# ModelTC/Dipoorlet

Measured on AMD Instinct MI355X. Metric: calibration images/sec (whole node) + achieved HBM GB/s, ResNet-50 ONNX N=1024, -A hist, higher is better.
Workload: dtype f32; 1 GPU; ResNet-50 ONNX activation set (T=123, 26598376 fp32 elems/img), -A hist --bins 2048, N=1024 per GPU in 32 batches of 32: range pass + histogram pass + percentile clip; device=AMD Radeon Graphics (gfx950:sramecc+:xnack-), hist_checksum_ok=True, world_size_seen_by_backend=1

## Files before the change

### dipoorlet_amd/csrc/calib_kernels.hip

```cpp
#include "common.hpp"

#pragma clang fp contract(off)

namespace {

__device__ __forceinline__ void minmax_commit(const MinMaxOp& op, uint32_t slot, float* s_mn, float* s_mx, uint32_t* s_nan,
                                              uint32_t* __restrict__ min_enc, uint32_t* __restrict__ max_enc,
                                              uint32_t* __restrict__ nan_flag) {
    float mn = wave_min(op.mn), mx = wave_max(op.mx);
    uint32_t nn = __any(op.nan) ? 1u : 0u;
    const int w = threadIdx.x / kWave;
    if ((threadIdx.x & (kWave - 1)) == 0) {
        s_mn[w] = mn;
        s_mx[w] = mx;
        s_nan[w] = nn;
    }
    __syncthreads();
    if (threadIdx.x == 0) {
#pragma unroll
        for (int j = 1; j < kBlock / kWave; ++j) {
            mn = fminf(mn, s_mn[j]);
            mx = fmaxf(mx, s_mx[j]);
            nn |= s_nan[j];
        }
        if (mn <= mx) {
            atomicMin(min_enc + slot, enc_f32(mn));
            atomicMax(max_enc + slot, enc_f32(mx));
        }
        if (nn) atomicOr(nan_flag + slot, 1u);
    }
    __syncthreads();
}

__global__ __launch_bounds__(kBlock) void k_minmax(const dpl_work_item* __restrict__ items,
                                                    const uint32_t* __restrict__ bb,
                                                    const float* const* __restrict__ segs,
                                                    uint32_t* __restrict__ min_enc, uint32_t* __restrict__ max_enc,
                                                    uint32_t* __restrict__ nan_flag) {
    __shared__ float s_mn[kBlock / kWave], s_mx[kBlock / kWave];
    __shared__ uint32_t s_nan[kBlock / kWave];
    uint32_t k0, k1;
    block_items(bb, k0, k1);
    for (uint32_t k = k0; k < k1; ++k) {
        const dpl_work_item it = items[k];
        MinMaxOp op{INFINITY, -INFINITY, 0u};
        stream_span(segs[it.seg] + it.offset, it.count, op);
        minmax_commit(op, it.slot, s_mn, s_mx, s_nan, min_enc, max_enc, nan_flag);
    }
}

__global__ void k_minmax_init(uint32_t* mn, uint32_t* mx, uint32_t* nan, int64_t n) {
    int64_t i = (int64_t)blockIdx.x * blockDim.x + threadIdx.x;
    if (i < n) {
        mn[i] = 0xFFFFFFFFu;
        mx[i] = 0u;
        nan[i] = 0u;
    }
}

__device__ __forceinline__ void minmax_decode(uint32_t mn, uint32_t mx, uint32_t nan, float& omn, float& omx) {
    const bool bad = nan != 0u || mn == 0xFFFFFFFFu;
    omn = bad ? NAN : dec_f32(mn);
    omx = bad ? NAN : dec_f32(mx);
}

__global__ void k_minmax_finalize(const uint32_t* mn, const uint32_t* mx, const uint32_t* nan, int64_t n,
                                  float* omn, float* omx) {
    int64_t i = (int64_t)blockIdx.x * blockDim.x + threadIdx.x;
    if (i < n) minmax_decode(mn[i], mx[i], nan[i], omn[i], omx[i]);
}

__global__ void k_minmax_encode(const float* mn, const float* mx, int64_t n, uint32_t* emn, uint32_t* emx,
                                uint32_t* nan) {
    int64_t i = (int64_t)blockIdx.x * blockDim.x + threadIdx.x;
    if (i < n) {
        const bool bad = (mn[i] != mn[i]) || (mx[i] != mx[i]);
        emn[i] = bad ? 0xFFFFFFFFu : enc_f32(mn[i]);
        emx[i] = bad ? 0u : enc_f32(mx[i]);
        nan[i] = bad ? 1u : 0u;
    }
}

__device__ __forceinline__ float hist_edge(int i, float step, float first) {
    return __fadd_rn(__fmul_rn((float)i, step), first);
}

template <bool kFast>
struct HistOp {
    uint32_t* lds;
    float first, last, step, inv, denom;
    int last_bin;
    float fbins;
    uint32_t nonzero;
    __device__ __forceinline__ void operator()(float x) {
        const float a = fabsf(x);
        const bool nz = (a != 0.0f);
        nonzero += nz;
        if (kFast) {
            if (nz && (a <= last)) {
                const int i = (int)__fmul_rn(a, inv);
                const uint32_t dec = (a < __fmul_rn((float)i, step)) ? 0xFFFFFFFCu : 0u;
                atomicAdd(reinterpret_cast<uint32_t*>(reinterpret_cast<char*>(lds) + (((uint32_t)i << 2) + dec)), 1u);
            }
            return;
        }
        int i;
        if (kFast) {
            i = (int)__fmul_rn(a, inv);
            i = i > last_bin ? last_bin : i;
            i -= (a < __fmul_rn((float)i, step)) ? 1 : 0;
        } else {
            i = (int)__fmul_rn(__fdiv_rn(__fsub_rn(a, first), denom), fbins);
            i = i > last_bin ? last_bin : i;
            i = i < 0 ? 0 : i;
            i -= (a < hist_edge(i, step, first)) ? 1 : 0;
            i += (i != last_bin && a >= hist_edge(i + 1, step, first)) ? 1 : 0;
        }
        if (nz && (a <= last)) atomicAdd(lds + i, 1u);
    }
};

template <bool kFast>
__device__ __forceinline__ void hist_op_init(HistOp<kFast>& op, const dpl_hist_range& r, int bins, uint32_t* lds) {
    op.lds = lds;
    op.first = r.first;
    op.last = r.last;
    op.step = r.step;
    op.inv = r.inv;
    op.denom = __fsub_rn(r.last, r.first);
    op.last_bin = bins - 1;
    op.fbins = (float)bins;
    op.nonzero = 0u;
}

struct HistLds {
    static __host__ __device__ uint32_t* s_nz(uint32_t* counters, int bins) { return counters + bins + 1; }
    static __host__ __device__ uint32_t* end(uint32_t* counters, int bins) { return s_nz(counters, bins) + kBlock / kWave; }
    static __host__ __device__ size_t bytes(int bins) { return ((size_t)bins + 1 + kBlock / kWave) * sizeof(uint32_t); }
};

template <class Count>
__device__ __forceinline__ void hist_flush(uint32_t nonzero, const dpl_work_item& it, const dpl_hist_range& r, int bins,
                                           Count* __restrict__ hist, uint32_t* lds, uint32_t* s_nz) {
    const uint32_t nzw = wave_sum(nonzero);
    if ((threadIdx.x & (kWave - 1)) == 0) s_nz[threadIdx.x / kWave] = nzw;
    __syncthreads();
    if (threadIdx.x == 0) {
        uint32_t nzb = 0;
        for (int k = 0; k < kBlock / kWave; ++k) nzb += s_nz[k];
        const uint32_t z = it.count - nzb;
        if (z) atomicAdd(lds + r.zero_bin, z);
        const uint32_t top = lds[bins];
        if (top) atomicAdd(lds + bins - 1, top);
    }
    __syncthreads();
    Count* __restrict__ out = hist + (uint64_t)it.slot * (uint64_t)bins;
    for (int b = threadIdx.x; b < bins; b += kBlock) {
        const uint32_t c = lds[b];
        if (c) {
            if constexpr (sizeof(Count) == 8)
                atomicAdd(reinterpret_cast<unsigned long long*>(out + b), (unsigned long long)c);
            else
                atomicAdd(out + b, c);
        }
    }
}

template <bool kFast>
__device__ __forceinline__ void hist_body(const dpl_work_item& it, const float* const* __restrict__ segs,
                                          const dpl_hist_range& r, int bins, uint64_t* __restrict__ hist,
                                          uint32_t* lds, uint32_t* s_nz) {
    HistOp<kFast> op;
    hist_op_init(op, r, bins, lds);
    stream_span(segs[it.seg] + it.offset, it.count, op);
    hist_flush(op.nonzero, it, r, bins, hist, lds, s_nz);
}

__global__ __launch_bounds__(kBlock) void k_abs_hist(const dpl_work_item* __restrict__ items,
                                                      const uint32_t* __restrict__ bb,
                                                      const float* const* __restrict__ segs,
                                                      const dpl_hist_range* __restrict__ ranges, int bins,
                                                      uint64_t* __restrict__ hist) {
    extern __shared__ __attribute__((aligned(16))) uint32_t lds[];
    uint32_t* s_nz = HistLds::s_nz(lds, bins);
    uint32_t k0, k1;
    block_items(bb, k0, k1);
    for (uint32_t k = k0; k < k1; ++k) {
        const dpl_work_item it = items[k];
        const dpl_hist_range r = ranges[it.slot];
        if (r.status != 0u) continue;
        for (int b = threadIdx.x; b <= bins; b += kBlock) lds[b] = 0u;
        __syncthreads();
        if (r.exact_div)
            hist_body<false>(it, segs, r, bins, hist, lds, s_nz);
        else
            hist_body<true>(it, segs, r, bins, hist, lds, s_nz);
        __syncthreads();
    }
}

__device__ __forceinline__ float py_max(float a, float b) { return (b > a) ? b : a; }
__device__ __forceinline__ float py_min(float a, float b) { return (b < a) ? b : a; }

__device__ __forceinline__ dpl_hist_range hist_range_of(float gmin, float gmax, int bins) {
    dpl_hist_range r;
    const float dmax = py_max(gmax, -gmin);
    float first = 0.0f, last = dmax;
    r.dmax = dmax;
    r.status = 0u;
    if (!(fabsf(last) <= 3.402823466e+38f) || last < first) r.status = 1u;
    if (first == last) {
        first = -0.5f;
        last = 0.5f;
    }
    const float delta = __fsub_rn(last, first);
    const float fb = (float)bins;
    r.first = first;
    r.last = last;
    r.step = __fdiv_rn(delta, fb);
    r.inv = __fmul_rn(__fdiv_rn(fb, delta), 1.000001f);
    if (r.status == 0u) {
        const float e1 = hist_edge(1, r.step, first);
        const float el = hist_edge(bins - 1, r.step, first);
        const float el2 = hist_edge(bins - 2 > 0 ? bins - 2 : 0, r.step, first);
        if (!(r.step > 0.0f) || !(e1 > first) || !(last > el) || (bins > 2 && !(el > el2))) r.status = 2u;
    }
    r.exact_div = (first != 0.0f || !(fabsf(r.inv) <= 3.402823466e+38f) || r.step < 1.0e-30f) ? 1u : 0u;
    {
        const float a = 0.0f;
        float t = __fmul_rn(__fdiv_rn(__fsub_rn(a, first), delta), fb);
        int b = (int)t;
        b = b > bins - 1 ? bins - 1 : b;
        b = b < 0 ? 0 : b;
        if (a < hist_edge(b, r.step, first)) --b;
        if (b != bins - 1 && a >= hist_edge(b + 1, r.step, first)) ++b;
        r.zero_bin = (uint32_t)(b < 0 ? 0 : b);
    }
    return r;
}

__global__ void k_hist_prepare(const float* __restrict__ gmin, const float* __restrict__ gmax, int64_t n, int bins,
                               dpl_hist_range* __restrict__ out) {
    int64_t i = (int64_t)blockIdx.x * blockDim.x + threadIdx.x;
    if (i >= n) return;
    out[i] = hist_range_of(gmin[i], gmax[i], bins);
}

struct SpecEntry {
    dpl_hist_range* snap;
    uint32_t* flags;
    uint32_t* counts;
    SpecEntry(const void* d_entry, int64_t n_slots)
        : snap((dpl_hist_range*)d_entry), flags((uint32_t*)(snap + n_slots)), counts((uint32_t*)((char*)d_entry + counts_offset(n_slots))) {}
    static uint64_t counts_offset(int64_t n_slots) {
        return (((uint64_t)n_slots * (sizeof(dpl_hist_range) + sizeof(uint32_t))) + 15ull) & ~15ull;
    }
    static uint64_t bytes(int64_t n_slots, int bins) { return counts_offset(n_slots) + (uint64_t)n_slots * (uint64_t)bins * sizeof(uint32_t); }
};

__global__ __launch_bounds__(kBlock) void k_hist_snapshot(const uint32_t* __restrict__ mn, const uint32_t* __restrict__ mx,
                                                           const uint32_t* __restrict__ nan, int64_t n, int bins,
                                                           dpl_hist_range* __restrict__ snap, uint32_t* __restrict__ flags,
                                                           uint32_t* __restrict__ counts) {
    const int64_t i = (int64_t)blockIdx.x * blockDim.x + threadIdx.x;
    const int64_t stride = (int64_t)gridDim.x * blockDim.x;
    if (i < n) {
        float gmin, gmax;
        minmax_decode(mn[i], mx[i], nan[i], gmin, gmax);
        snap[i] = hist_range_of(gmin, gmax, bins);
        flags[i] = 0u;
    }
    const int64_t total = n * (int64_t)bins;
    for (int64_t j = i; j < total; j += stride) counts[j] = 0u;
}

template <bool kFast>
struct MinMaxHistOp {
    MinMaxOp m;
    HistOp<kFast> h;
    __device__ __forceinline__ void operator()(float x) {
        m(x);
        h(x);
    }
};

template <bool kFast>
__device__ __forceinline__ void minmax_hist_body(const dpl_work_item& it, const float* const* __restrict__ segs,
                                                 const dpl_hist_range& r, int bins, uint32_t* __restrict__ counts,
                                                 uint32_t* lds, uint32_t* s_nz, MinMaxOp& m) {
    MinMaxHistOp<kFast> op;
    op.m = m;
    hist_op_init(op.h, r, bins, lds);
    stream_span(segs[it.seg] + it.offset, it.count, op);
    m = op.m;
    hist_flush(op.h.nonzero, it, r, bins, counts, lds, s_nz);
}

struct MinMaxHistLds {
    static __host__ __device__ float* s_mn(uint32_t* base, int bins) { return reinterpret_cast<float*>(HistLds::end(base, bins)); }
    static __host__ __device__ float* s_mx(uint32_t* base, int bins) { return s_mn(base, bins) + kBlock / kWave; }
    static __host__ __device__ uint32_t* s_nan(uint32_t* base, int bins) {
        return reinterpret_cast<uint32_t*>(s_mx(base, bins) + kBlock / kWave);
    }
    static __host__ __device__ size_t bytes(int bins) { return HistLds::bytes(bins) + 3 * (kBlock / kWave) * sizeof(uint32_t); }
};

__global__ __launch_bounds__(kBlock) void k_minmax_hist(const dpl_work_item* __restrict__ items,
                                                         const uint32_t* __restrict__ bb,
                                                         const float* const* __restrict__ segs,
                                                         uint32_t* __restrict__ min_enc, uint32_t* __restrict__ max_enc,
                                                         uint32_t* __restrict__ nan_flag,
                                                         const dpl_hist_range* __restrict__ snap, int bins,
                                                         uint32_t* __restrict__ counts) {
    extern __shared__ __attribute__((aligned(16))) uint32_t lds_mh[];
    uint32_t* s_nz = HistLds::s_nz(lds_mh, bins);
    float* s_mn = MinMaxHistLds::s_mn(lds_mh, bins);
    float* s_mx = MinMaxHistLds::s_mx(lds_mh, bins);
    uint32_t* s_nan = MinMaxHistLds::s_nan(lds_mh, bins);
    uint32_t k0, k1;
    block_items(bb, k0, k1);
    for (uint32_t k = k0; k < k1; ++k) {
        const dpl_work_item it = items[k];
        const dpl_hist_range r = snap[it.slot];
        MinMaxOp m{INFINITY, -INFINITY, 0u};
        if (r.status != 0u) {
            stream_span(segs[it.seg] + it.offset, it.count, m);
        } else {
            for (int b = threadIdx.x; b <= bins; b += kBlock) lds_mh[b] = 0u;
            __syncthreads();
            if (r.exact_div)
                minmax_hist_body<false>(it, segs, r, bins, counts, lds_mh, s_nz, m);
            else
                minmax_hist_body<true>(it, segs, r, bins, counts, lds_mh, s_nz, m);
        }
        minmax_commit(m, it.slot, s_mn, s_mx, s_nan, min_enc, max_enc, nan_flag);
    }
}

__global__ __launch_bounds__(kBlock) void k_hist_resolve(const dpl_hist_range* __restrict__ snap,
                                                          const dpl_hist_range* __restrict__ fin,
                                                          const uint32_t* __restrict__ counts, const uint64_t* __restrict__ elems,
                                                          int bins, uint64_t* __restrict__ hist, uint32_t* __restrict__ flags,
                                                          unsigned long long* __restrict__ stats) {
    const uint32_t t = blockIdx.x;
    const uint32_t* a = reinterpret_cast<const uint32_t*>(snap + t);
    const uint32_t* b = reinterpret_cast<const uint32_t*>(fin + t);
    bool same = true;
#pragma unroll
    for (int w = 0; w < (int)(sizeof(dpl_hist_range) / 4); ++w) same = same && (a[w] == b[w]);
    const uint32_t status = fin[t].status;
    const bool valid = same && status == 0u;
    if (threadIdx.x == 0) {
        flags[t] = valid ? 1u : (status != 0u ? 2u : 0u);
        if (stats) {
            const unsigned long long e = elems[t];
            atomicAdd(stats + 0, 1ull);
            atomicAdd(stats + 2, e);
            if (valid) {
                atomicAdd(stats + 1, 1ull);
                atomicAdd(stats + 3, e);
            }
        }
    }
    if (!valid) return;
    const uint32_t* __restrict__ row = counts + (uint64_t)t * (uint64_t)bins;
    uint64_t* __restrict__ out = hist + (uint64_t)t * (uint64_t)bins;
    for (int j = threadIdx.x; j < bins; j += kBlock) {
        const uint32_t c = row[j];
        if (c) out[j] += (uint64_t)c;
    }
}

__device__ __forceinline__ uint64_t shfl_up_u64(uint64_t v, int d) {
    const uint32_t lo = __shfl_up((uint32_t)v, d, kWave), hi = __shfl_up((uint32_t)(v >> 32), d, kWave);
    return ((uint64_t)hi << 32) | lo;
}

__device__ __forceinline__ void rest_prefix(const uint64_t* __restrict__ elems, const uint32_t* __restrict__ flags, int n_tensors,
                                            uint64_t* P, uint64_t* s_tot) {
    const int per = (n_tensors + kBlock - 1) / kBlock;
    const int t0 = (int)threadIdx.x * per;
    uint64_t mine = 0;
    for (int j = 0; j < per; ++j) {
        const int t = t0 + j;
        if (t < n_tensors && flags[t] == 0u) mine += elems[t];
    }
    uint64_t incl = mine;
    const int lane = threadIdx.x & (kWave - 1), wv = threadIdx.x / kWave;
#pragma unroll
    for (int o = 1; o < kWave; o <<= 1) {
        const uint64_t up = shfl_up_u64(incl, o);
        if (lane >= o) incl += up;
    }
    if (lane == kWave - 1) s_tot[wv] = incl;
    __syncthreads();
    uint64_t run = incl - mine;
    for (int w = 0; w < wv; ++w) run += s_tot[w];
    for (int j = 0; j < per; ++j) {
        const int t = t0 + j;
        if (t < n_tensors) {
            P[t] = run;
            if (flags[t] == 0u) run += elems[t];
        }
    }
    if (threadIdx.x == kBlock - 1) P[n_tensors] = run;
    __syncthreads();
}

__device__ __forceinline__ void rest_cut(const uint64_t* P, int n_tensors, uint64_t G, uint64_t b, uint64_t& cut, int& at) {
    const uint64_t total = P[n_tensors], q = total / G, rem = total % G;
    const uint64_t target = (b >= G) ? total : q * b + (rem * b) / G;
    if (target >= total) {
        cut = total;
        at = n_tensors;
        return;
    }
    int lo = 1, hi = n_tensors;
    while (lo < hi) {
        const int mid = (lo + hi) >> 1;
        if (P[mid] > target) hi = mid; else lo = mid + 1;
    }
    at = lo - 1;
    cut = P[lo - 1] + ((target - P[lo - 1]) & ~1023ull);
}

struct RestPrefixLds {
    static __host__ __device__ uint64_t* P(uint32_t* base) { return reinterpret_cast<uint64_t*>(base); }
    static __host__ __device__ uint64_t* s_tot(uint32_t* base, int n_tensors) { return P(base) + n_tensors + 1; }
    static __host__ __device__ size_t bytes(int64_t n_tensors) { return ((size_t)n_tensors + 1 + kBlock / kWave) * sizeof(uint64_t); }
};

struct RestLds {
    static __host__ __device__ uint32_t* counters(uint32_t* base, int n_tensors) {
        return reinterpret_cast<uint32_t*>(RestPrefixLds::s_tot(base, n_tensors) + kBlock / kWave);
    }
    static __host__ __device__ size_t bytes(int64_t n_tensors, int bins) { return RestPrefixLds::bytes(n_tensors) + HistLds::bytes(bins); }
};

__global__ __launch_bounds__(kBlock) void k_abs_hist_rest(const uint64_t* __restrict__ elems, const uint32_t* __restrict__ flags,
                                                           int n_tensors, const float* const* __restrict__ segs,
                                                           const dpl_hist_range* __restrict__ ranges, int bins,
                                                           uint64_t* __restrict__ hist) {
    extern __shared__ __attribute__((aligned(16))) uint32_t lds_rest[];
    uint64_t* P = RestPrefixLds::P(lds_rest);
    uint64_t* s_tot = RestPrefixLds::s_tot(lds_rest, n_tensors);
    uint32_t* lds = RestLds::counters(lds_rest, n_tensors);
    uint32_t* s_nz = HistLds::s_nz(lds, bins);
    rest_prefix(elems, flags, n_tensors, P, s_tot);
    if (P[n_tensors] == 0) return;
    uint64_t cut[2];
    int at[2];
    rest_cut(P, n_tensors, gridDim.x, blockIdx.x, cut[0], at[0]);
    rest_cut(P, n_tensors, gridDim.x, (uint64_t)blockIdx.x + 1, cut[1], at[1]);
    uint64_t pos = cut[0];
    const uint64_t end = cut[1];
    int t = at[0];
    while (pos < end) {
        while (P[t + 1] <= pos) ++t;
        const uint64_t stop = P[t + 1] < end ? P[t + 1] : end;
        dpl_work_item it;
        it.offset = pos - P[t];
        it.count = (uint32_t)(stop - pos);
        it.seg = (uint32_t)t;
        it.slot = (uint32_t)t;
        it.reserved = 0u;
        const dpl_hist_range r = ranges[t];
        for (int b = threadIdx.x; b <= bins; b += kBlock) lds[b] = 0u;
        __syncthreads();
        if (r.exact_div)
            hist_body<false>(it, segs, r, bins, hist, lds, s_nz);
        else
            hist_body<true>(it, segs, r, bins, hist, lds, s_nz);
        __syncthreads();
        pos = stop;
    }
}

__global__ __launch_bounds__(kBlock) void k_hist_spec_cuts(const uint64_t* __restrict__ elems, const uint32_t* __restrict__ flags,
                                                            int n_tensors, uint64_t* __restrict__ cuts) {
    extern __shared__ __attribute__((aligned(16))) uint32_t lds_cuts[];
    uint64_t* P = RestPrefixLds::P(lds_cuts);
    uint64_t* s_tot = RestPrefixLds::s_tot(lds_cuts, n_tensors);
    rest_prefix(elems, flags, n_tensors, P, s_tot);
    if (threadIdx.x != 0) return;
    uint64_t cut = 0;
    int at = 0;
    if (P[n_tensors] != 0) rest_cut(P, n_tensors, gridDim.x, blockIdx.x, cut, at);
    cuts[blockIdx.x] = cut;
    if (blockIdx.x + 1 == gridDim.x) cuts[gridDim.x] = P[n_tensors];
}

__device__ __forceinline__ void store_bin_clip(int found, float gmin, float gmax, int bins, float* __restrict__ clip) {
    float lo = gmin, hi = gmax;
    if (found >= 0) {
        const float dmax = py_max(-gmin, gmax);
        const float cv = __fmul_rn((float)found + 0.5f, __fdiv_rn(dmax, (float)bins));
        lo = py_max(-cv, gmin);
        hi = py_min(cv, gmax);
    }
    clip[0] = lo;
    clip[1] = hi;
}

__global__ __launch_bounds__(kWave) void k_hist_percentile(const uint64_t* __restrict__ hist,
                                                            const float* __restrict__ gmin_a,
                                                            const float* __restrict__ gmax_a, int bins,
                                                            double threshold, float* __restrict__ clip) {
    const int slot = blockIdx.x;
    const int lane = threadIdx.x;
    const uint64_t* h = hist + (uint64_t)slot * bins;
    unsigned long long tot = 0;
    for (int b = lane; b < bins; b += kWave) tot += h[b];
#pragma unroll
    for (int o = 32; o > 0; o >>= 1) tot += __shfl_xor(tot, o, kWave);
    const double total = (double)(long long)tot;
    const float gmin = gmin_a[slot], gmax = gmax_a[slot];
    double accum = 0.0;
    int found = -1;
    uint64_t raw_next = lane < bins ? h[lane] : 0ull;
    for (int base = 0; base < bins && found < 0; base += kWave) {
        const int b = base + lane;
        const double hv = (b < bins) ? (double)(float)(long long)raw_next / total : 0.0;
        raw_next = (b + kWave < bins) ? h[b + kWave] : 0ull;
        const int lim = (bins - base) < kWave ? (bins - base) : kWave;
        const int h_lo = __double2loint(hv), h_hi = __double2hiint(hv);
        uint64_t reached = 0;
        if (lim == kWave) {
#pragma unroll
            for (int j = 0; j < kWave; ++j) {
                accum += __hiloint2double(__builtin_amdgcn_readlane(h_hi, j), __builtin_amdgcn_readlane(h_lo, j));
                reached |= (accum >= threshold) ? (1ull << j) : 0ull;
            }
        } else {
            for (int j = 0; j < lim; ++j) {
                accum += __hiloint2double(__builtin_amdgcn_readlane(h_hi, j), __builtin_amdgcn_readlane(h_lo, j));
                reached |= (accum >= threshold) ? (1ull << j) : 0ull;
            }
        }
        if (reached) found = base + __builtin_ctzll(reached);
    }
    if (lane == 0) store_bin_clip(found, gmin, gmax, bins, clip + 2 * slot);
}

constexpr double kKlEps = 1e-4;

__device__ __forceinline__ uint32_t kl_live_below(const uint64_t* __restrict__ mask, const uint32_t* __restrict__ bcnt, uint32_t x) {
    const uint32_t k = x >> 6;
    return bcnt[k] + (uint32_t)__popcll(mask[k] & ((1ull << (x & 63u)) - 1ull));
}

struct KlLds {
    static __host__ __device__ uint32_t nblk(int bins) { return ((uint32_t)bins + 63u) >> 6; }
    static __host__ __device__ uint64_t* mask(uint64_t* cs, int bins) { return cs + bins + 1; }
    static __host__ __device__ uint64_t* part(uint64_t* cs, int bins) { return mask(cs, bins) + nblk(bins) + 1; }
    static __host__ __device__ uint32_t* bcnt(uint64_t* cs, int bins) { return reinterpret_cast<uint32_t*>(part(cs, bins) + kBlock); }
    static __host__ __device__ size_t bytes(int bins) {
        return ((size_t)bins + 1 + nblk(bins) + 1 + kBlock) * sizeof(uint64_t) + ((size_t)nblk(bins) + 1) * sizeof(uint32_t);
    }
};

__global__ __launch_bounds__(kBlock) void k_hist_kl(const uint64_t* __restrict__ hist, int bins, int levels, int n_chunks,
                                                     double* __restrict__ div) {
    extern __shared__ __attribute__((aligned(16))) uint64_t kl_lds[];
    const uint32_t nblk = KlLds::nblk(bins);
    uint64_t* cs = kl_lds;
    uint64_t* mask = KlLds::mask(kl_lds, bins);
    uint64_t* part = KlLds::part(kl_lds, bins);
    uint32_t* bcnt = KlLds::bcnt(kl_lds, bins);
    const uint32_t tid = threadIdx.x, lane = tid & (kWave - 1), wave = tid / kWave;
    const uint32_t slot = blockIdx.x / (uint32_t)n_chunks, chunk = blockIdx.x % (uint32_t)n_chunks;
    const uint64_t* __restrict__ h = hist + (uint64_t)slot * (uint64_t)bins;
    double* __restrict__ out = div + (uint64_t)slot * ((uint64_t)bins + 1u);
    const uint32_t L = (uint32_t)levels, C = (uint32_t)n_chunks, nb = (uint32_t)bins;

    {
        const uint32_t per = (nb + kBlock - 1) / kBlock;
        const uint32_t b0 = tid * per < nb ? tid * per : nb, b1 = b0 + per < nb ? b0 + per : nb;
        uint64_t s = 0;
        for (uint32_t b = b0; b < b1; ++b) s += h[b];
        part[tid] = s;
        for (uint32_t k = wave; k < nblk; k += kBlock / kWave) {
            const uint32_t b = k * kWave + lane;
            const uint64_t m = __ballot(b < nb && h[b] != 0ull);
            if (lane == 0) mask[k] = m;
        }
        if (tid == 0) mask[nblk] = 0ull;
        __syncthreads();
        uint64_t off = 0;
        for (uint32_t j = 0; j < (uint32_t)kBlock; ++j) off += j < tid ? part[j] : 0ull;
        for (uint32_t b = b0; b < b1; ++b) {
            cs[b] = off;
            off += h[b];
        }
        if (tid == kBlock - 1) cs[nb] = off;
        for (uint32_t k = tid; k <= nblk; k += kBlock) {
            uint32_t a = 0;
            for (uint32_t j = 0; j < nblk; ++j) a += j < k ? (uint32_t)__popcll(mask[j]) : 0u;
            bcnt[k] = a;
        }
        __syncthreads();
    }
    for (uint32_t i = chunk + tid * C; i < L; i += kBlock * C) out[i] = INFINITY;

    const uint64_t N = cs[nb];
    const double dN = (double)(long long)N;
    const uint32_t first = L + (chunk + C - L % C) % C;
    for (uint32_t i = first + wave * C; i <= nb; i += (kBlock / kWave) * C) {
        const uint64_t csi = cs[i];
        const uint64_t outl = N - csi;
        const uint32_t s_last = (uint32_t)(((uint64_t)(L - 1u) * i) / L);
        const uint32_t woke = (csi == cs[i - 1] && outl != 0ull) ? 1u : 0u;
        const uint32_t n1p = kl_live_below(mask, bcnt, i) + woke;
        const uint32_t n1q = n1p - ((csi == cs[s_last] && outl != 0ull) ? 1u : 0u);
        double res = INFINITY;
        if (n1p != 0u && n1q != 0u) {
            const uint32_t zp = i - n1p, zq = i - n1q;
            const double e1p = kKlEps * (double)zp / (double)n1p;
            const double e1q = kKlEps * (double)zq / (double)n1q;
            if (e1p < 1.0 && e1q < 1.0) {
                const double Sp = dN - (double)n1p * e1p + (double)zp * kKlEps;
                const double Sq = (double)(long long)csi - (double)n1q * e1q + (double)zq * kKlEps;
                double acc = 0.0;
                for (uint32_t b = lane; b < i; b += kWave) {
                    uint64_t pb = cs[b + 1] - cs[b];
                    if (b == i - 1u) pb += outl;
                    if (pb != 0ull) {
                        const uint32_t g = ((b + 1u) * L - 1u) / i;
                        const uint32_t s0 = (g * i) / L, s1 = ((g + 1u) * i) / L;
                        const uint64_t G = cs[s1] - cs[s0];
                        double qs = kKlEps;
                        if (G != 0ull) {
                            const uint32_t live = kl_live_below(mask, bcnt, s1) - kl_live_below(mask, bcnt, s0) + (s1 == i ? woke : 0u);
                            qs = (double)(long long)G / (double)live - e1q;
                        }
                        const double P = ((double)(long long)pb - e1p) / Sp, Q = qs / Sq;
                        acc += P * log(P / Q);
                    }
                }
                acc = wave_sum(acc);
                const double Pz = kKlEps / Sp, Qz = kKlEps / Sq;
                res = acc + (double)zp * (Pz * log(Pz / Qz));
            }
        }
        if (lane == 0) out[i] = res;
    }
}

__global__ __launch_bounds__(kWave) void k_hist_kl_pick(const double* __restrict__ div, const float* __restrict__ gmin_a,
                                                         const float* __restrict__ gmax_a, int bins, int32_t* __restrict__ best,
                                                         float* __restrict__ clip) {
    const int slot = blockIdx.x;
    const int lane = threadIdx.x;
    const double* __restrict__ d = div + (uint64_t)slot * ((uint64_t)bins + 1u);
    double bv = INFINITY;
    int bi = -1;
    for (int i = lane; i <= bins; i += kWave) {
        const double v = d[i];
        if (v < bv) {
            bv = v;
            bi = i;
        }
    }
#pragma unroll
    for (int o = 32; o > 0; o >>= 1) {
        const double ov = __shfl_xor(bv, o, kWave);
        const int oi = __shfl_xor(bi, o, kWave);
        if (ov < bv || (ov == bv && oi >= 0 && (bi < 0 || oi < bi))) {
            bv = ov;
            bi = oi;
        }
    }
    if (lane == 0) {
        best[slot] = bi;
        store_bin_clip(bi >= 0 ? bi - 1 : -1, gmin_a[slot], gmax_a[slot], bins, clip + 2 * slot);
    }
}

constexpr int kGridUniform = DPL_GRID_UNIFORM, kGridE4M3 = DPL_GRID_E4M3;

struct QmseLds {
    static __host__ __device__ uint64_t* part(double* hd, int bins) { return reinterpret_cast<uint64_t*>(hd + bins); }
    static __host__ __device__ size_t bytes(int bins) { return (size_t)bins * sizeof(double) + (kBlock / kWave) * sizeof(uint64_t); }
};

template <int GRID>
__global__ __launch_bounds__(kBlock) void k_hist_qmse(const uint64_t* __restrict__ hist, int bins, int first, int top, int n_chunks,
                                                       double* __restrict__ err) {
    extern __shared__ __attribute__((aligned(16))) double qm_lds[];
    double* hd = qm_lds;
    uint64_t* part = QmseLds::part(qm_lds, bins);
    const uint32_t tid = threadIdx.x, lane = tid & (kWave - 1), wave = tid / kWave;
    const uint32_t slot = blockIdx.x / (uint32_t)n_chunks, chunk = blockIdx.x % (uint32_t)n_chunks;
    const uint64_t* __restrict__ h = hist + (uint64_t)slot * (uint64_t)bins;
    double* __restrict__ out = err + (uint64_t)slot * ((uint64_t)bins + 1u);
    const uint32_t F = (uint32_t)first, C = (uint32_t)n_chunks, nb = (uint32_t)bins;

    uint64_t s = 0;
    for (uint32_t b = tid; b < nb; b += kBlock) {
        const uint64_t v = h[b];
        s += v;
        hd[b] = (double)(long long)v;
    }
#pragma unroll
    for (int o = 32; o > 0; o >>= 1) s += __shfl_xor(s, o, kWave);
    if (lane == 0) part[wave] = s;
    __syncthreads();
    uint64_t N = 0;
#pragma unroll
    for (int w = 0; w < kBlock / kWave; ++w) N += part[w];

    for (uint32_t i = chunk + tid * C; i < F; i += kBlock * C) out[i] = INFINITY;

    constexpr double unit = GRID == kGridE4M3 ? 512.0 : 1.0;
    const double dtop = GRID == kGridE4M3 ? 448.0 : (double)top;
    const double atop = unit * dtop;
    const double norm = (double)(long long)N * (4.0 * atop * atop);
    for (uint32_t i = F + chunk + wave * C; i <= nb; i += (kBlock / kWave) * C) {
        const double t = (double)(2u * i - 1u);
        const double rt = 1.0 / (unit * t);
        double acc = 0.0;
        if (N != 0ull) {
            for (uint32_t b = lane; b < nb; b += kWave) {
                const double hb = hd[b];
                if (hb != 0.0) {
                    const double a = (double)(2u * b + 1u) * atop;
                    const double v = fmin(a * rt, dtop);
                    double q;
                    if (GRID == kGridE4M3) {
                        int e = (int)((__double_as_longlong(v) >> 52) & 0x7FF) - 1023;
                        e = e < -6 ? -6 : e;
                        const double istep = __longlong_as_double((long long)(1023 + 3 - e) << 52);
                        const double step512 = __longlong_as_double((long long)(1023 + 9 - 3 + e) << 52);
                        q = rint(v * istep) * step512;
                    } else {
                        q = rint(v);
                    }
                    const double dt = a - q * t;
                    acc += hb * (dt * dt);
                }
            }
            acc = wave_sum(acc);
        }
        if (lane == 0) out[i] = N != 0ull ? acc / norm : INFINITY;
    }
}

inline int check_bins(const char* who, int bins) {
    if (bins < 1 || bins > DPL_MAX_BINS) {
        snprintf(g_err, sizeof(g_err), "%s: bins must be in [1, %d]", who, DPL_MAX_BINS);
        return -2;
    }
    return 0;
}

inline int check_spec_geometry(const char* who, int64_t n_slots, int64_t n_blocks) {
    const bool slots_ok = n_slots > 0 && n_slots <= DPL_HIST_SPEC_MAX_TENSORS;
    if (slots_ok && n_blocks > 0 && n_blocks <= 0x7FFFFFFFll) return 0;
    snprintf(g_err, sizeof(g_err), "%s: %s", who, slots_ok ? "n_blocks out of range" : "n_slots must be in [1, DPL_HIST_SPEC_MAX_TENSORS]");
    return -2;
}

inline int candidate_chunks(const char* who, int64_t n_slots, int64_t n_cand, int64_t& chunks) {
    chunks = (1024 + n_slots - 1) / n_slots;
    if (chunks > n_cand / 8) chunks = n_cand / 8;
    if (chunks < 1) chunks = 1;
    if (n_slots * chunks > 0x7FFFFFFFll) {
        snprintf(g_err, sizeof(g_err), "%s: too many slots", who);
        return -2;
    }
    return 0;
}

}

extern "C" {

int dpl_minmax_init(uint32_t* d_min_enc, uint32_t* d_max_enc, uint32_t* d_nan, int64_t n_slots, dpl_stream_t s) {
    if (n_slots <= 0) return 0;
    hipLaunchKernelGGL(k_minmax_init, dim3(grid_for(n_slots, 256)), dim3(256), 0, (hipStream_t)s, d_min_enc,
                       d_max_enc, d_nan, n_slots);
    DPL_LAUNCH_CHECK("k_minmax_init");
    return 0;
}

int dpl_minmax_accumulate(const dpl_work_item* d_items, int64_t n_items, const uint32_t* d_block_begin,
                          int64_t n_blocks, const float* const* d_seg_ptrs, uint32_t* d_min_enc,
                          uint32_t* d_max_enc, uint32_t* d_nan, dpl_stream_t s) {
    if (n_items <= 0) return 0;
    if (int e = check_blocks("dpl_minmax_accumulate", n_items, d_block_begin, n_blocks)) return e;
    hipLaunchKernelGGL(k_minmax, dim3((unsigned)n_blocks), dim3(kBlock), 0, (hipStream_t)s, d_items, d_block_begin,
                       d_seg_ptrs, d_min_enc, d_max_enc, d_nan);
    DPL_LAUNCH_CHECK("k_minmax");
    return 0;
}

int dpl_minmax_finalize(const uint32_t* d_min_enc, const uint32_t* d_max_enc, const uint32_t* d_nan,
                        int64_t n_slots, float* d_min, float* d_max, dpl_stream_t s) {
    if (n_slots <= 0) return 0;
    hipLaunchKernelGGL(k_minmax_finalize, dim3(grid_for(n_slots, 256)), dim3(256), 0, (hipStream_t)s, d_min_enc,
                       d_max_enc, d_nan, n_slots, d_min, d_max);
    DPL_LAUNCH_CHECK("k_minmax_finalize");
    return 0;
}

int dpl_minmax_encode(const float* d_min, const float* d_max, int64_t n_slots, uint32_t* d_min_enc,
                      uint32_t* d_max_enc, uint32_t* d_nan, dpl_stream_t s) {
    if (n_slots <= 0) return 0;
    hipLaunchKernelGGL(k_minmax_encode, dim3(grid_for(n_slots, 256)), dim3(256), 0, (hipStream_t)s, d_min, d_max,
                       n_slots, d_min_enc, d_max_enc, d_nan);
    DPL_LAUNCH_CHECK("k_minmax_encode");
    return 0;
}

int dpl_hist_prepare(const float* d_min, const float* d_max, int64_t n_slots, int bins, dpl_hist_range* d_ranges,
                     dpl_stream_t s) {
    if (int e = check_bins("dpl_hist_prepare", bins)) return e;
    if (n_slots <= 0) return 0;
    hipLaunchKernelGGL(k_hist_prepare, dim3(grid_for(n_slots, 64)), dim3(64), 0, (hipStream_t)s, d_min, d_max,
                       n_slots, bins, d_ranges);
    DPL_LAUNCH_CHECK("k_hist_prepare");
    return 0;
}

int dpl_abs_hist_accumulate(const dpl_work_item* d_items, int64_t n_items, const uint32_t* d_block_begin,
                            int64_t n_blocks, const float* const* d_seg_ptrs, const dpl_hist_range* d_ranges,
                            int bins, uint64_t* d_hist, dpl_stream_t s) {
    if (int e = check_bins("dpl_abs_hist_accumulate", bins)) return e;
    if (n_items <= 0) return 0;
    if (int e = check_blocks("dpl_abs_hist_accumulate", n_items, d_block_begin, n_blocks)) return e;
    hipLaunchKernelGGL(k_abs_hist, dim3((unsigned)n_blocks), dim3(kBlock), HistLds::bytes(bins), (hipStream_t)s, d_items,
                       d_block_begin, d_seg_ptrs, d_ranges, bins, d_hist);
    DPL_LAUNCH_CHECK("k_abs_hist");
    return 0;
}

uint64_t dpl_hist_spec_entry_bytes(int64_t n_slots, int bins) {
    if (n_slots < 0 || bins < 1 || bins > DPL_MAX_BINS) return 0;
    return SpecEntry::bytes(n_slots, bins);
}

int dpl_minmax_hist_accumulate(const dpl_work_item* d_items, int64_t n_items, const uint32_t* d_block_begin,
                               int64_t n_blocks, const float* const* d_seg_ptrs, uint32_t* d_min_enc, uint32_t* d_max_enc,
                               uint32_t* d_nan, int64_t n_slots, int bins, void* d_entry, dpl_stream_t s) {
    if (int e = check_bins("dpl_minmax_hist_accumulate", bins)) return e;
    if (!d_entry || ((uintptr_t)d_entry & 15u)) return fail_msg("dpl_minmax_hist_accumulate: d_entry must be 16-byte aligned");
    if (n_slots <= 0 || n_slots > 0x7FFFFFFFll) return fail_msg("dpl_minmax_hist_accumulate: n_slots out of range");
    if (n_items <= 0) return 0;
    if (int e = check_blocks("dpl_minmax_hist_accumulate", n_items, d_block_begin, n_blocks)) return e;
    const SpecEntry entry(d_entry, n_slots);
    int64_t zb = grid_for(n_slots * (int64_t)bins, kBlock * 8);
    if (zb < grid_for(n_slots, kBlock)) zb = grid_for(n_slots, kBlock);
    if (zb > 1024) zb = 1024;
    hipLaunchKernelGGL(k_hist_snapshot, dim3((unsigned)zb), dim3(kBlock), 0, (hipStream_t)s, d_min_enc, d_max_enc, d_nan,
                       n_slots, bins, entry.snap, entry.flags, entry.counts);
    DPL_LAUNCH_CHECK("k_hist_snapshot");
    hipLaunchKernelGGL(k_minmax_hist, dim3((unsigned)n_blocks), dim3(kBlock), MinMaxHistLds::bytes(bins), (hipStream_t)s, d_items,
                       d_block_begin, d_seg_ptrs, d_min_enc, d_max_enc, d_nan, entry.snap, bins, entry.counts);
    DPL_LAUNCH_CHECK("k_minmax_hist");
    return 0;
}

int dpl_hist_spec_accumulate(void* d_entry, const uint64_t* d_elems, int64_t n_slots, int64_t n_blocks,
                             const float* const* d_seg_ptrs, const dpl_hist_range* d_ranges, int bins, uint64_t* d_hist,
                             uint64_t* d_stats, dpl_stream_t s) {
    if (int e = check_bins("dpl_hist_spec_accumulate", bins)) return e;
    if (!d_entry || ((uintptr_t)d_entry & 15u)) return fail_msg("dpl_hist_spec_accumulate: d_entry must be 16-byte aligned");
    if (int e = check_spec_geometry("dpl_hist_spec_accumulate", n_slots, n_blocks)) return e;
    const SpecEntry entry(d_entry, n_slots);
    hipLaunchKernelGGL(k_hist_resolve, dim3((unsigned)n_slots), dim3(kBlock), 0, (hipStream_t)s, entry.snap, d_ranges, entry.counts,
                       d_elems, bins, d_hist, entry.flags, (unsigned long long*)d_stats);
    DPL_LAUNCH_CHECK("k_hist_resolve");
    hipLaunchKernelGGL(k_abs_hist_rest, dim3((unsigned)n_blocks), dim3(kBlock), RestLds::bytes(n_slots, bins), (hipStream_t)s, d_elems,
                       entry.flags, (int)n_slots, d_seg_ptrs, d_ranges, bins, d_hist);
    DPL_LAUNCH_CHECK("k_abs_hist_rest");
    return 0;
}

int dpl_hist_spec_cuts(const void* d_entry, const uint64_t* d_elems, int64_t n_slots, int64_t n_blocks, uint64_t* d_cuts,
                       dpl_stream_t s) {
    if (!d_entry || !d_cuts) return fail_msg("dpl_hist_spec_cuts: null argument");
    if (int e = check_spec_geometry("dpl_hist_spec_cuts", n_slots, n_blocks)) return e;
    hipLaunchKernelGGL(k_hist_spec_cuts, dim3((unsigned)n_blocks), dim3(kBlock), RestPrefixLds::bytes(n_slots), (hipStream_t)s, d_elems,
                       SpecEntry(d_entry, n_slots).flags, (int)n_slots, d_cuts);
    DPL_LAUNCH_CHECK("k_hist_spec_cuts");
    return 0;
}

int dpl_hist_percentile(const uint64_t* d_hist, const float* d_min, const float* d_max, int64_t n_slots, int bins,
                        double threshold, float* d_clip, dpl_stream_t s) {
    if (n_slots <= 0) return 0;
    hipLaunchKernelGGL(k_hist_percentile, dim3((unsigned)n_slots), dim3(kWave), 0, (hipStream_t)s, d_hist, d_min,
                       d_max, bins, threshold, d_clip);
    DPL_LAUNCH_CHECK("k_hist_percentile");
    return 0;
}

int dpl_hist_kl(const uint64_t* d_hist, const float* d_min, const float* d_max, int64_t n_slots, int bins, int levels,
                double* d_div, int32_t* d_best, float* d_clip, dpl_stream_t s) {
    if (int e = check_bins("dpl_hist_kl", bins)) return e;
    if (levels < 2 || levels > bins) return fail_msg("dpl_hist_kl: levels must be in [2, bins]");
    if (n_slots <= 0) return 0;
    int64_t chunks;
    if (int e = candidate_chunks("dpl_hist_kl", n_slots, (int64_t)bins - levels + 1, chunks)) return e;
    hipLaunchKernelGGL(k_hist_kl, dim3((unsigned)(n_slots * chunks)), dim3(kBlock), KlLds::bytes(bins), (hipStream_t)s, d_hist, bins,
                       levels, (int)chunks, d_div);
    DPL_LAUNCH_CHECK("k_hist_kl");
    hipLaunchKernelGGL(k_hist_kl_pick, dim3((unsigned)n_slots), dim3(kWave), 0, (hipStream_t)s, d_div, d_min, d_max, bins,
                       d_best, d_clip);
    DPL_LAUNCH_CHECK("k_hist_kl_pick");
    return 0;
}

int dpl_hist_qmse(const uint64_t* d_hist, const float* d_min, const float* d_max, int64_t n_slots, int bins, int first, int grid,
                  int top, double* d_err, int32_t* d_best, float* d_clip, dpl_stream_t s) {
    if (int e = check_bins("dpl_hist_qmse", bins)) return e;
    if (first < 1 || first > bins) return fail_msg("dpl_hist_qmse: first must be in [1, bins]");
    if (grid != DPL_GRID_UNIFORM && grid != DPL_GRID_E4M3) return fail_msg("dpl_hist_qmse: grid must be DPL_GRID_UNIFORM or DPL_GRID_E4M3");
    if (grid == DPL_GRID_UNIFORM && (top < 1 || top > 32767)) return fail_msg("dpl_hist_qmse: top must be in [1, 32767] on the uniform grid");
    if (grid == DPL_GRID_E4M3 && top != 0) return fail_msg("dpl_hist_qmse: top must be 0 on the E4M3 grid (its largest value is 448)");
    if (n_slots <= 0) return 0;
    int64_t chunks;
    if (int e = candidate_chunks("dpl_hist_qmse", n_slots, (int64_t)bins - first + 1, chunks)) return e;
    const size_t lds = QmseLds::bytes(bins);
    const dim3 wgs((unsigned)(n_slots * chunks));
    if (grid == DPL_GRID_E4M3)
        hipLaunchKernelGGL(k_hist_qmse<kGridE4M3>, wgs, dim3(kBlock), lds, (hipStream_t)s, d_hist, bins, first, top, (int)chunks, d_err);
    else
        hipLaunchKernelGGL(k_hist_qmse<kGridUniform>, wgs, dim3(kBlock), lds, (hipStream_t)s, d_hist, bins, first, top, (int)chunks, d_err);
    DPL_LAUNCH_CHECK("k_hist_qmse");
    hipLaunchKernelGGL(k_hist_kl_pick, dim3((unsigned)n_slots), dim3(kWave), 0, (hipStream_t)s, d_err, d_min, d_max, bins,
                       d_best, d_clip);
    DPL_LAUNCH_CHECK("k_hist_kl_pick");
    return 0;
}

}
```

Baseline: 58750 images/s.

## Fuse speculative histogram resolve into rest-histogram kernel, batch row adds

Merges the per-tensor resolve kernel into the rest-histogram kernel. Each block now recomputes the snapshot-versus-final verdict inline for the prefix sum, adds validated speculative count rows in a grid-stride loop, and then processes its share of unresolved data. This drops one kernel launch and the dependency between the two kernels. Row accumulation is batched with 8 loads in flight per thread. The cost is that every block re-reads all snapshot and range records during the prefix, and the rest histogram work now waits behind each block's share of row adds.

Measured after the change: 59030 images/s (median of 2 runs). Within noise of the previous version (+0.5%).

```diff
diff --git a/dipoorlet_amd/csrc/calib_kernels.hip b/dipoorlet_amd/csrc/calib_kernels.hip
--- a/dipoorlet_amd/csrc/calib_kernels.hip
+++ b/dipoorlet_amd/csrc/calib_kernels.hip
@@ -337,37 +337,35 @@
     }
 }
 
-__global__ __launch_bounds__(kBlock) void k_hist_resolve(const dpl_hist_range* __restrict__ snap,
-                                                          const dpl_hist_range* __restrict__ fin,
-                                                          const uint32_t* __restrict__ counts, const uint64_t* __restrict__ elems,
-                                                          int bins, uint64_t* __restrict__ hist, uint32_t* __restrict__ flags,
-                                                          unsigned long long* __restrict__ stats) {
-    const uint32_t t = blockIdx.x;
+__device__ __forceinline__ uint32_t spec_verdict(const dpl_hist_range* __restrict__ snap, const dpl_hist_range* __restrict__ fin,
+                                                 uint32_t t) {
     const uint32_t* a = reinterpret_cast<const uint32_t*>(snap + t);
     const uint32_t* b = reinterpret_cast<const uint32_t*>(fin + t);
-    bool same = true;
-#pragma unroll
-    for (int w = 0; w < (int)(sizeof(dpl_hist_range) / 4); ++w) same = same && (a[w] == b[w]);
+    uint32_t diff = 0u;
+#pragma unroll
+    for (int w = 0; w < (int)(sizeof(dpl_hist_range) / 4); ++w) diff |= a[w] ^ b[w];
     const uint32_t status = fin[t].status;
-    const bool valid = same && status == 0u;
-    if (threadIdx.x == 0) {
-        flags[t] = valid ? 1u : (status != 0u ? 2u : 0u);
-        if (stats) {
-            const unsigned long long e = elems[t];
-            atomicAdd(stats + 0, 1ull);
-            atomicAdd(stats + 2, e);
-            if (valid) {
-                atomicAdd(stats + 1, 1ull);
-                atomicAdd(stats + 3, e);
-            }
-        }
-    }
-    if (!valid) return;
-    const uint32_t* __restrict__ row = counts + (uint64_t)t * (uint64_t)bins;
-    uint64_t* __restrict__ out = hist + (uint64_t)t * (uint64_t)bins;
-    for (int j = threadIdx.x; j < bins; j += kBlock) {
-        const uint32_t c = row[j];
-        if (c) out[j] += (uint64_t)c;
+    return status != 0u ? 2u : (diff == 0u ? 1u : 0u);
+}
+
+constexpr int kRowTrip = 8;
+__device__ __forceinline__ void spec_add_row(const uint32_t* __restrict__ row, uint64_t* __restrict__ out, int bins) {
+    for (int base = (int)threadIdx.x; base < bins; base += kBlock * kRowTrip) {
+        uint32_t c[kRowTrip];
+        uint64_t h[kRowTrip];
+#pragma unroll
+        for (int k = 0; k < kRowTrip; ++k) {
+            const int j = base + k * kBlock, jj = j < bins ? j : bins - 1;
+            c[k] = row[jj];
+            h[k] = out[jj];
+        }
+#pragma unroll
+        for (int k = 0; k < kRowTrip; ++k) asm volatile("" : "+v"(c[k]), "+v"(h[k]));
+#pragma unroll
+        for (int k = 0; k < kRowTrip; ++k) {
+            const int j = base + k * kBlock;
+            if (j < bins && c[k]) out[j] = h[k] + (uint64_t)c[k];
+        }
     }
 }
 
@@ -376,14 +374,20 @@
     return ((uint64_t)hi << 32) | lo;
 }
 
-__device__ __forceinline__ void rest_prefix(const uint64_t* __restrict__ elems, const uint32_t* __restrict__ flags, int n_tensors,
-                                            uint64_t* P, uint64_t* s_tot) {
+template <class ToRead>
+__device__ __forceinline__ void rest_prefix(const uint64_t* __restrict__ elems, int n_tensors, uint64_t* P, uint64_t* s_tot,
+                                            ToRead to_read) {
     const int per = (n_tensors + kBlock - 1) / kBlock;
     const int t0 = (int)threadIdx.x * per;
     uint64_t mine = 0;
     for (int j = 0; j < per; ++j) {
         const int t = t0 + j;
-        if (t < n_tensors && flags[t] == 0u) mine += elems[t];
+        if (t < n_tensors) {
+            const uint64_t e = elems[t];
+            const uint64_t share = to_read(t) ? e : 0ull;
+            P[t] = share;
+            mine += share;
+        }
     }
     uint64_t incl = mine;
     const int lane = threadIdx.x & (kWave - 1), wv = threadIdx.x / kWave;
@@ -399,8 +403,9 @@
     for (int j = 0; j < per; ++j) {
         const int t = t0 + j;
         if (t < n_tensors) {
+            const uint64_t share = P[t];
             P[t] = run;
-            if (flags[t] == 0u) run += elems[t];
+            run += share;
         }
     }
     if (threadIdx.x == kBlock - 1) P[n_tensors] = run;
@@ -437,16 +442,33 @@
     static __host__ __device__ size_t bytes(int64_t n_tensors, int bins) { return RestPrefixLds::bytes(n_tensors) + HistLds::bytes(bins); }
 };
 
-__global__ __launch_bounds__(kBlock) void k_abs_hist_rest(const uint64_t* __restrict__ elems, const uint32_t* __restrict__ flags,
-                                                           int n_tensors, const float* const* __restrict__ segs,
-                                                           const dpl_hist_range* __restrict__ ranges, int bins,
-                                                           uint64_t* __restrict__ hist) {
+__global__ __launch_bounds__(kBlock) void k_hist_spec(const dpl_hist_range* __restrict__ snap, uint32_t* __restrict__ flags,
+                                                       const uint32_t* __restrict__ counts, const uint64_t* __restrict__ elems,
+                                                       int n_tensors, const float* const* __restrict__ segs,
+                                                       const dpl_hist_range* __restrict__ ranges, int bins,
+                                                       uint64_t* __restrict__ hist, unsigned long long* __restrict__ stats) {
     extern __shared__ __attribute__((aligned(16))) uint32_t lds_rest[];
     uint64_t* P = RestPrefixLds::P(lds_rest);
     uint64_t* s_tot = RestPrefixLds::s_tot(lds_rest, n_tensors);
     uint32_t* lds = RestLds::counters(lds_rest, n_tensors);
     uint32_t* s_nz = HistLds::s_nz(lds, bins);
-    rest_prefix(elems, flags, n_tensors, P, s_tot);
+    rest_prefix(elems, n_tensors, P, s_tot, [&](int t) { return spec_verdict(snap, ranges, (uint32_t)t) == 0u; });
+    for (uint32_t t = blockIdx.x; t < (uint32_t)n_tensors; t += gridDim.x) {
+        const uint32_t verdict = spec_verdict(snap, ranges, t);
+        if (threadIdx.x == 0) {
+            flags[t] = verdict;
+            if (stats) {
+                const unsigned long long e = elems[t];
+                atomicAdd(stats + 0, 1ull);
+                atomicAdd(stats + 2, e);
+                if (verdict == 1u) {
+                    atomicAdd(stats + 1, 1ull);
+                    atomicAdd(stats + 3, e);
+                }
+            }
+        }
+        if (verdict == 1u) spec_add_row(counts + (uint64_t)t * (uint64_t)bins, hist + (uint64_t)t * (uint64_t)bins, bins);
+    }
     if (P[n_tensors] == 0) return;
     uint64_t cut[2];
     int at[2];
@@ -481,7 +503,7 @@
     extern __shared__ __attribute__((aligned(16))) uint32_t lds_cuts[];
     uint64_t* P = RestPrefixLds::P(lds_cuts);
     uint64_t* s_tot = RestPrefixLds::s_tot(lds_cuts, n_tensors);
-    rest_prefix(elems, flags, n_tensors, P, s_tot);
+    rest_prefix(elems, n_tensors, P, s_tot, [&](int t) { return flags[t] == 0u; });
     if (threadIdx.x != 0) return;
     uint64_t cut = 0;
     int at = 0;
@@ -867,12 +889,10 @@
     if (!d_entry || ((uintptr_t)d_entry & 15u)) return fail_msg("dpl_hist_spec_accumulate: d_entry must be 16-byte aligned");
     if (int e = check_spec_geometry("dpl_hist_spec_accumulate", n_slots, n_blocks)) return e;
     const SpecEntry entry(d_entry, n_slots);
-    hipLaunchKernelGGL(k_hist_resolve, dim3((unsigned)n_slots), dim3(kBlock), 0, (hipStream_t)s, entry.snap, d_ranges, entry.counts,
-                       d_elems, bins, d_hist, entry.flags, (unsigned long long*)d_stats);
-    DPL_LAUNCH_CHECK("k_hist_resolve");
-    hipLaunchKernelGGL(k_abs_hist_rest, dim3((unsigned)n_blocks), dim3(kBlock), RestLds::bytes(n_slots, bins), (hipStream_t)s, d_elems,
-                       entry.flags, (int)n_slots, d_seg_ptrs, d_ranges, bins, d_hist);
-    DPL_LAUNCH_CHECK("k_abs_hist_rest");
+    hipLaunchKernelGGL(k_hist_spec, dim3((unsigned)n_blocks), dim3(kBlock), RestLds::bytes(n_slots, bins), (hipStream_t)s, entry.snap,
+                       entry.flags, entry.counts, d_elems, (int)n_slots, d_seg_ptrs, d_ranges, bins, d_hist,
+                       (unsigned long long*)d_stats);
+    DPL_LAUNCH_CHECK("k_hist_spec");
     return 0;
 }
 
```
